# byvfx/go-raytracing

Hardware: AMD Instinct MI355X
Metric: Msamples/sec (pixels x SPP / s) (higher is better)
Workload: dtype f32; 1 GPU; cornell-lucy 1200x675 500spp depth 5; scene=cornell-lucy, width=1200, height=675, spp=500, max_depth=5, parallelism=tiles-rr1, buckets=836, blas=sah, nodes=fp32, triangles=280000, bvh_nodes=60240, bvh_nodes8=0, image_finite=True

## Files before the change

### go-raytracing_amd/__init__.py

```python
from __future__ import annotations

import ctypes as C
import os
from typing import Optional, Sequence

import numpy as np

PKG_DIR = os.path.dirname(os.path.abspath(__file__))
LIB_DIR = os.path.join(PKG_DIR, os.environ.get("RTGPU_LIB_DIR", "lib"))
REPO_DIR = os.path.dirname(PKG_DIR)
ASSET_DIR = os.path.join(REPO_DIR, "assets")

RT_OK = 0
RT_OPT_BLAS_BUILDER, RT_OPT_TLAS_BUILDER, RT_OPT_NODE_FORMAT = 1, 2, 3
RT_OPT_BATCH_SLOTS, RT_OPT_REFILL, RT_OPT_MAX_BLOCKS, RT_OPT_STREAMS = 4, 5, 6, 7
RT_OPT_VOLUMES = 8
RT_VOLUMES_LIFTED, RT_VOLUMES_IN_BVH = 0, 1
RT_OPT_BVH4_COLLAPSE = 9
RT_COLLAPSE_SAH, RT_COLLAPSE_GREEDY = 0, 1
RT_BLAS_REFERENCE, RT_BLAS_SAH, RT_BLAS_DEVICE = 0, 1, 2
RT_NODES_FP32, RT_NODES_QUANT8, RT_NODES_WIDE8 = 0, 1, 2
RT_OPT_DEALING, RT_OPT_DEAL_FIRST = 10, 11
RT_OPT_TAIL = 12
RT_OPT_OVERLAP = 13
RT_OPT_LIFT_PRIMS = 14
RT_PRIMS_LIFTED, RT_PRIMS_IN_BVH = 0, 1
RT_DEAL_STATIC, RT_DEAL_DYNAMIC = 0, 1
STATUS = {0: "RT_OK", -1: "RT_ERR_INVALID", -2: "RT_ERR_UNSUPPORTED", -3: "RT_ERR_HIP", -4: "RT_ERR_OOM",
          -5: "RT_ERR_NO_SCENE", -6: "RT_ERR_DEVICE"}

RT_SPHERE, RT_QUAD, RT_TRIANGLE, RT_PLANE, RT_LIST, RT_BVH_NODE, RT_BVH_LEAF = 1, 2, 3, 4, 5, 6, 7
RT_TRANSLATE, RT_ROTATE_X, RT_ROTATE_Y, RT_ROTATE_Z, RT_SCALE, RT_VOLUME = 8, 9, 10, 11, 12, 13
RT_CIRCLE = 14
RT_LAMBERTIAN, RT_METAL, RT_DIELECTRIC, RT_DIFFUSE_LIGHT, RT_ISOTROPIC = 1, 2, 3, 4, 5
RT_TEX_SOLID, RT_TEX_CHECKER, RT_TEX_NOISE, RT_TEX_IMAGE = 1, 2, 3, 4


class RtHittable(C.Structure):
    _fields_ = [("kind", C.c_int32), ("material", C.c_int32), ("a", C.c_int32), ("b", C.c_int32),
                ("bbox", C.c_double * 6), ("p", C.c_double * 16)]
# ... 149 lines not shown
        p.use_sky_gradient, p.phantom_hdri, p.camera_max_depth = camera.use_sky_gradient, camera.phantom_hdri, camera.max_depth
    for k, v in sky.items():
        if k == "background":
            p.background = (C.c_double * 3)(*[float(x) for x in v])
        elif k in ("use_sky_gradient", "phantom_hdri", "camera_max_depth"):
            setattr(p, k, int(v))
        else:
            raise TypeError(f"unknown rt_ray_color_params field {k!r}")
    return p


class RtWorkCounts(C.Structure):
    _fields_ = [(n, C.c_uint64) for n in ("samples", "rays", "shadow_rays", "node_visits", "sphere_tests",
                                          "quad_tests", "tri_tests", "plane_tests", "instance_visits",
                                          "volume_tests", "material_fetches", "env_lookups",
                                          "instance_box_tests", "stack_spills")]


class RtKernelTimes(C.Structure):
    _fields_ = [("extend_ms", C.c_double), ("shade_ms", C.c_double), ("shadow_ms", C.c_double),
                ("extend_launches", C.c_int32), ("shade_launches", C.c_int32), ("shadow_launches", C.c_int32),
                ("twins", C.c_int32)]


class RtSceneInfo(C.Structure):
    _fields_ = [(n, C.c_int32) for n in ("nodes", "leaves", "refs", "spheres", "quads", "triangles", "planes",
                                         "instances", "blases", "volumes", "materials", "textures", "lights",
                                         "stack_needed", "tlas_depth", "blas_depth")] + [("device_bytes", C.c_int64)] + \
        [("node_format", C.c_int32), ("nodes8", C.c_int32)]


# ... 557 lines not shown
    def set_collapse(self, collapse: str):
        self.set_option(RT_OPT_BVH4_COLLAPSE, {"sah": RT_COLLAPSE_SAH, "greedy": RT_COLLAPSE_GREEDY}[collapse])

    def set_schedule(self, batch_slots: int = 0, refill: int = 0, max_blocks: int = 0, streams: int = 0):
        self.set_option(RT_OPT_BATCH_SLOTS, batch_slots)
        self.set_option(RT_OPT_REFILL, refill)
        self.set_option(RT_OPT_MAX_BLOCKS, max_blocks)
        self.set_option(RT_OPT_STREAMS, streams)

    def set_tail(self, paths: int = 0):
        self.set_option(RT_OPT_TAIL, paths)

    def set_overlap(self, mode: int = 0):
        self.set_option(RT_OPT_OVERLAP, mode)

    def measure_read_bandwidth(self, nbytes: int = 4 << 30, reps: int = 10) -> float:
        gbs = C.c_double(0.0)
        self._check(self._lib.rt_measure_read_bandwidth(self._h, C.c_uint64(nbytes), reps, C.byref(gbs)))
        return float(gbs.value)

    def set_kernel_timing(self, enable: bool = True):
        self._check(self._lib.rt_set_kernel_timing(self._h, 1 if enable else 0))

    def last_kernel_times(self) -> dict:
        t = RtKernelTimes()
        self._check(self._lib.rt_last_kernel_times(self._h, C.byref(t)))
        return {n: getattr(t, n) for n, _ in RtKernelTimes._fields_}

    def tonemap(self, accum: np.ndarray, spp: int) -> np.ndarray:
        h, w = accum.shape[:2]
# ... 158 lines not shown
```

### go-raytracing_amd/csrc/api.cpp

```cpp
#include <hip/hip_runtime.h>

#include <algorithm>
#include <atomic>
#include <chrono>
#include <cstdio>
#include <cstdlib>
#include <cmath>
#include <cstring>
#include <string>
#include <thread>
#include <vector>

#include "../../include/rtgpu.h"
#include "dev_layout.h"
#include "build.h"
#include "flatten.h"
#include "probe.h"
#include "query.h"
#include "ray_source.h"
#include "wavefront.h"
#include "wave_layout.h"
#include "denoise.h"
#include "denoise_var.h"
#include "adaptive.h"
// ... 380 lines not shown
  hipStream_t sts[kMaxTwins] = {st};
  for (int t = 1; t < kMaxTwins; ++t) sts[t] = ctx->twin_st[t - 1];
  for (int t = 0; t < nt; ++t) {
    WaveArgs& a = as[t];
    bind_twin(a, static_cast<float4*>(ctx->wstate.p), static_cast<uint32_t*>(ctx->wq.p),
              static_cast<const uint32_t*>(ctx->wpix.p), static_cast<double*>(ctx->wacc.p),
              static_cast<uint32_t*>(ctx->wspill.p), lay.tw[t], lit);
    if (run.feat) feat_acc[t] = static_cast<double*>(ctx->wfacc.p) + lay.tw[t].pix_off * kFeatFloats;
    if (run.mom_out) mom_acc[t] = static_cast<double*>(ctx->wmacc.p) + lay.tw[t].pix_off * kMomFloats;
    a.seed = p->seed;
    a.max_depth = p->max_depth;
    a.counters = static_cast<unsigned long long*>(ctx->counters.p);
    a.err = static_cast<int*>(ctx->errflag.p);
    a.refill = knobs.refill;
    a.nee_probe = run.probing ? 1u : 0u;
    a.spill_lanes = spill.lanes;
    a.spill_cap = spill.cap;
    a.out_pixels = run.rays ? run.rays->num_rays : uint32_t(dc.width) * uint32_t(dc.height);
    ctx->twin_args[t] = a;
  }
  ctx->num_twins = nt;
  WavePlan plan{};
  plan.spp = spp;
  plan.samples_per_batch = bs.spb;
  plan.sample_offset = uint32_t(p->sample_offset);
  plan.max_depth = p->max_depth;
  if (run.feat) {
    plan.max_depth = 1;
    plan.feat_acc = feat_acc;
  }
// ... 371 lines not shown
    return RT_OK;
  }
  if (key == RT_OPT_REFILL) {
    if (value < 0 || value > 64) return set_err(ctx, RT_ERR_INVALID, "refill must be 0 (default) or 1..64");
    ctx->wopt.refill = value;
    return RT_OK;
  }
  if (key == RT_OPT_STREAMS) {
    if (value < 0 || value > kMaxTwins) return set_err(ctx, RT_ERR_INVALID, "streams must be 0 (default) or 1..4");
    ctx->wopt.streams = value;
    return RT_OK;
  }
  if (key == RT_OPT_OVERLAP) {
    if (value < 0 || value > 2) return set_err(ctx, RT_ERR_INVALID, "overlap must be 0 (default), 1 (off) or 2 (on)");
    ctx->wopt.overlap = value;
    return RT_OK;
  }
  if (key == RT_OPT_TAIL) {
    if (value < 0) return set_err(ctx, RT_ERR_INVALID, "bad tail option");
    ctx->wopt.tail = value;
    return RT_OK;
  }
  if (key == RT_OPT_MAX_BLOCKS) {
    if (value < 0) return set_err(ctx, RT_ERR_INVALID, "bad max blocks");
    ctx->wopt.blocks = value;
    return RT_OK;
  }
  if (key == RT_OPT_DEALING) {
    if (value != RT_DEAL_STATIC && value != RT_DEAL_DYNAMIC) return set_err(ctx, RT_ERR_INVALID, "bad dealing mode");
    ctx->opt_dealing = value;
// ... 783 lines not shown
void fill_counts(const unsigned long long* c, rt_work_counts* out) {
  out->samples = c[0];
  out->rays = c[1];
  out->shadow_rays = c[2];
  out->node_visits = c[3];
  out->sphere_tests = c[4];
  out->quad_tests = c[5];
  out->tri_tests = c[6];
  out->plane_tests = c[7];
  out->instance_visits = c[8];
  out->volume_tests = c[9];
  out->material_fetches = c[10];
  out->env_lookups = c[11];
  out->instance_box_tests = c[12];
  out->stack_spills = c[13];
}
}

int rt_count_work_by_kernel(rt_ctx* ctx, const rt_camera_desc* cam, const rt_render_params* params,
                            rt_work_counts* out) {
  if (!ctx || !cam || !out) return RT_ERR_INVALID;
  HIPCHK(hipSetDevice(ctx->device));
  unsigned long long c[CNT_WORDS] = {0};
  double ms = 0.0;
  int rc = render_impl(ctx, cam, params, nullptr, RenderRun{ctx->stream, &ms, c});
  if (rc) return rc;
  for (int k = 0; k < 3; ++k) fill_counts(c + k * CNT_BLOCK, out + k);
  return RT_OK;
}

// ... 473 lines not shown
```

### go-raytracing_amd/csrc/dev_layout.h

```cpp
#pragma once
#include <stdint.h>
#if !defined(__HIPCC__) && !defined(__host__)
#define __host__
#define __device__
#endif

namespace rtg {

enum : uint32_t {
  ITEM_NODE = 0u,
  ITEM_LEAF = 1u,
  ITEM_INSTANCE = 2u,
  ITEM_INST_END = 3u,
  ITEM_TRI1 = 4u,
  ITEM_WQUAD = 8u,
  ITEM_WSPHERE = 9u,
  ITEM_WINST = 10u,
  ITEM_LREF = 11u,
  ITEM_WTRI1 = 12u,
};
constexpr int ITEM_SHIFT = 28;
constexpr uint32_t ITEM_MASK = (1u << ITEM_SHIFT) - 1u;
constexpr int kInlineTriMax = 4;
__host__ __device__ inline uint32_t tri_leaf_item(uint32_t first, int n) {
// ... 300 lines not shown
  int32_t num_vol_refs;
  int32_t shade_kind;
  int32_t needs_uv;
  int32_t quant_nodes;
  int32_t dfs_order;
  int32_t wide_nodes;
  uint32_t root8;
  const DNode8* nodes8;
  const uint32_t* litems;
  const DWTri* wtris;
  uint32_t n_nodes, n_leaves, n_refs, n_spheres, n_quads, n_tris, n_instances, n_blas, n_volumes, n_circles;
  uint32_t n_nodes8, n_litems, n_wtris;
  int32_t num_prim_recs;
  const DPrimRec* prim_recs;
};

struct DCamera {
  float center[3];
  float pixel00[3];
  float du[3], dv[3];
  float disk_u[3], disk_v[3];
  float background[3];
  int32_t defocus;
  int32_t use_sky;
  int32_t phantom;
  int32_t cam_max_depth;
  int32_t width, height;
  int32_t slow, free_cam;
  float c_orig[3], c_dir[3];
  float la_orig[3], la_dir[3];
// ... 18 lines not shown
```

### go-raytracing_amd/csrc/device_common.h

```cpp
#pragma once
#include <hip/hip_runtime.h>
#include <stdint.h>
#include "dev_layout.h"

namespace rtg {

#ifdef RTG_GUARD
__device__ unsigned int rtg_guard_rec[4];
__device__ __forceinline__ void rtg_guard_note(int site, uint32_t i, uint32_t n) {
  if (atomicAdd(&rtg_guard_rec[0], 1u) == 0u) {
    rtg_guard_rec[1] = uint32_t(site);
    rtg_guard_rec[2] = i;
    rtg_guard_rec[3] = n;
  }
}
__device__ __forceinline__ uint32_t rtg_gix(uint32_t i, uint32_t n, int site) {
  if (i >= n) {
    rtg_guard_note(site, i, n);
    return n ? n - 1u : 0u;
  }
  return i;
}
#define GIX(i, n, site) rtg_gix(uint32_t(i), uint32_t(n), site)
#else
// ... 272 lines not shown
  const bool cc = closed_kind(kind), bc = closed_kind(bkind);
  if (cc != bc) return cc;
  const int rc = obj_rank(sc, refpos), rb = obj_rank(sc, brefpos);
  bool later;
  if (rc == rb) {
    if (primpos == bprimpos) return false;
    later = prim_rank(sc, kind, primpos) > prim_rank(sc, bkind, bprimpos);
  } else {
    later = rc > rb;
  }
  return cc ? later : !later;
}

struct Cnt {
  uint32_t rays, shadow, nodes, sph, quad, tri, plane, inst, vol, mat, env, ibox, spill;
};
__device__ __forceinline__ bool volume_flight(const DVolume& vol, V3 wd, bool h1, bool h2, float t1, float t2,
                                              float tmin, float tmax, int ntests, uint32_t key, uint32_t bounce,
                                              uint32_t dom, float& t_out) {
  if (!h1 || !h2) return false;
  if (t1 < tmin) t1 = tmin;
  if (t2 > tmax) t2 = tmax;
  if (t1 >= t2) return false;
  if (t1 < 0.0f) t1 = 0.0f;
  float rl = len(wd);
  float dist = (t2 - t1) * rl;
  float u = 0.0f;
  for (int p = 0; p < ntests; ++p) {
    float up = rnd(key, ctr(bounce, dom, uint32_t(vol.vol_id) * 4u + uint32_t(p)));
    u = up > u ? up : u;
// ... 363 lines not shown
  if (t < bt) return true;
  if (t == bt && bt < T.tmax) return tie_wins(sc, kind, refpos, primpos, S.hit_kind(), S.hit_refpos(), S.hit_primpos());
  return false;
}
__device__ __forceinline__ void take_hit(Trav& T, const TStack& S, float t, int kind, int idx, int refpos, int primpos) {
  T.bt = cull_widen(t);
  S.set_hit(kind, idx, refpos, primpos);
}
__device__ __forceinline__ Best trav_best(const Trav& T, const TStack& S) {
  Best b;
  b.t = best_t(T); b.inst = -1;
  b.kind = S.hit_kind(); b.idx = S.hit_idx(); b.refpos = S.hit_refpos(); b.primpos = S.hit_primpos();
  return b;
}

template <bool kAny, bool kCount, bool kWide = false>
__device__ __forceinline__ int trav_init(const DScene& sc, Trav& T, const TStack& S, V3 wo, V3 wd, float time,
                                         float tmin, float tmax, uint32_t key, uint32_t bounce, uint32_t voldom,
                                         Cnt& cnt) {
  S.set_time(time); T.tmin = tmin; T.tmax = tmax;
  T.key = key; T.bounce = bounce; T.voldom = voldom;
  T.bt = cull_widen(tmax);
  if (!kAny) S.set_hit(0, -1, 0, 0);
  for (int i = 0; i < sc.num_planes; ++i) {
    float t = 0.0f;
    if (kCount) cnt.plane++;
    if (plane_t(sc.planes[i], wo, wd, tmin, t)) {
      if (kAny) { if (t < tmax) return TRAV_ANYHIT; }
      else if (accept_hit(sc, t, PK_PLANE, -1 - i, 0, T, S)) take_hit(T, S, t, PK_PLANE, i, -1 - i, 0);
    }
  }
  T.cr = make_tray(wo, wd);
  S.save_world(wo, wd, T.cr.inv);
  S.set_cur_ref(-1); T.sp = 0;
  T.item = ITEM_NONE; T.lf = ITEM_NONE;
  float tn = 0.0f;
  if (sc.tlas.check_box &&
      !box_hit(sc.tlas.box[0], sc.tlas.box[1], sc.tlas.box[2], sc.tlas.box[3], sc.tlas.box[4], sc.tlas.box[5],
               T.cr, tmin, kAny ? tmax : T.bt, tn))
    return TRAV_DONE;
  T.item = kWide ? sc.root8 : sc.tlas.root_item;
  if ((T.item >> ITEM_SHIFT) != ITEM_NODE) {
    T.lf = T.item;
    T.item = item_is_leaf(T.lf) ? ITEM_NONE : ITEM_POP;
  }
  return TRAV_RUNNING;
}

template <bool kAny, bool kCount, bool kVol, bool kQuant = false, bool kWide = false, int kLdsN = 0>
__device__ __forceinline__ int trav_step(const DScene& sc, Trav& T, const TStack& S, Cnt& cnt, int* err) {
  const bool exact = kVol && !kAny && sc.dfs_order != 0;
  auto pop = [&]() -> uint32_t {
    for (;;) {
      if (T.sp == 0) return ITEM_NONE;
      --T.sp;
// ... 667 lines not shown
```

### go-raytracing_amd/csrc/wave_layout.h

```cpp
#pragma once
#include <algorithm>
#include <cstddef>
#include <cstdint>
#include <cstdlib>
#include <vector>

#include "wavefront.h"

namespace rtg {


struct WaveOptions {
  size_t slots = 0;
  int refill = 0;
  int blocks = 0;
  int tail = 0;
  int streams = 0;
  int overlap = 0;
};

struct WaveKnobs {
  int streams = 0;
  int overlap = 0;
  size_t slots = 0;
  int refill = 16;
  int max_blocks = 0;
  int debug_sync = 0;
  uint32_t tail_rays = 0;
  int tail_first = kTailFirstDefault;
};

struct WaveEnv {
  int streams, overlap, refill, max_blocks, tail_rays, tail_first, debug_sync;
  size_t slots;
};

inline WaveEnv read_wave_env() {
  auto num = [](const char* name, long unset) {
    const char* e = getenv(name);
    return e ? atol(e) : unset;
  };
  WaveEnv v{};
  v.streams = int(std::min<long>(kMaxTwins, std::max<long>(0, num("RTGPU_STREAMS", 0))));
  v.overlap = int(num("RTGPU_OVERLAP", 0));
  v.slots = size_t(std::max<long>(0, num("RTGPU_SLOTS", 0)));
  v.refill = int(std::min<long>(64, std::max<long>(1, num("RTGPU_REFILL", 16))));
  v.max_blocks = int(std::max<long>(0, num("RTGPU_MAX_BLOCKS", 0)));
  const long tail = num("RTGPU_TAIL_RAYS", -1);
  v.tail_rays = tail >= 0 ? int(tail) : kTailRaysDefault;
  v.tail_first = int(num("RTGPU_TAIL_FIRST", kTailFirstDefault));
  v.debug_sync = num("RTGPU_DEBUG_SYNC", 0) > 0 ? 1 : 0;
  return v;
}

inline const WaveEnv& wave_env() {
  static const WaveEnv env = read_wave_env();
  return env;
}

inline WaveKnobs resolve_knobs(const WaveOptions& opt, bool probing, const WaveEnv& env = wave_env()) {
  WaveKnobs k;
  k.streams = opt.streams ? opt.streams : env.streams;
  k.overlap = opt.overlap ? opt.overlap : env.overlap;
  k.slots = opt.slots ? opt.slots : env.slots;
  k.refill = opt.refill ? opt.refill : env.refill;
  k.max_blocks = opt.blocks ? opt.blocks : env.max_blocks;
  k.debug_sync = env.debug_sync;
  k.tail_rays = probing || opt.tail == 1 ? 0u : uint32_t(opt.tail > 1 ? opt.tail : env.tail_rays);
  k.tail_first = env.tail_first;
  return k;
}


constexpr int kDefaultTwins = 2;
constexpr uint64_t kThreeTwinSamples = uint64_t(1) << 26;
constexpr int kOverlapTwins = 2;

inline uint64_t tile_pixels(const std::vector<int4>& tiles) {
  uint64_t n = 0;
  for (const int4& tl : tiles) n += uint64_t(tl.z) * uint64_t(tl.w);
  return n;
}

inline bool use_overlap(const WaveKnobs& k, bool lit) { return lit && k.overlap == 2; }

inline int choose_twins(const WaveKnobs& k, bool shade_vol, bool overlap, uint64_t tile_px, int spp, size_t ntiles) {
  int automatic = shade_vol ? 1 : tile_px * uint64_t(std::max(1, spp)) > kThreeTwinSamples ? 3 : kDefaultTwins;
  if (overlap) automatic = std::min(automatic, kOverlapTwins);
  const int want = k.streams ? k.streams : automatic;
  return int(std::max<size_t>(1, std::min<size_t>(size_t(std::max(1, want)), ntiles)));
}

inline void deal_pixels(const std::vector<int4>& tiles, int width, int nt, std::vector<uint32_t>& out,
                        uint32_t twin_npix[kMaxTwins]) {
  out.clear();
  for (int t = 0; t < kMaxTwins; ++t) twin_npix[t] = 0;
  for (int t = 0; t < nt; ++t) {
    const size_t before = out.size();
    for (size_t k = size_t(t); k < tiles.size(); k += size_t(nt)) {
// ... 162 lines not shown
```

### go-raytracing_amd/csrc/wavefront.h

```cpp
#pragma once
#include <hip/hip_runtime.h>
#include <stdint.h>
#include "dev_layout.h"
#include "features.h"
#include "moments.h"

namespace rtg {

struct RaySource;

struct PathStream {
  float4* o;
  float4* d;
  float4* beta;
};

constexpr int kSlotF4 = 14;
constexpr int kSlotF4Dark = 8;

struct WaveArgs {
  PathStream s[2];
  float4* hit;
  float4* Lout;
  float4* sj_p;
// ... 8 lines not shown
  const uint32_t* pixels;
  uint32_t npix;
  double* acc;
  uint32_t seed;
  int32_t max_depth;
  unsigned long long* counters;
  int* err;
  int32_t refill;
  uint32_t nee_probe;
  uint32_t* spill;
  uint32_t* spill_sh;
  uint32_t spill_lanes;
  int32_t spill_cap;
  uint32_t slots;
  uint32_t out_pixels;
};

enum : int { CNT_STREAM0 = 0, CNT_STREAM1 = 32, CNT_SHADOW = 64, CNT_FETCH_EXT = 128, CNT_FETCH_SH = 384,
             CNT_SHADE_SEG = 896, CNT_WORDS_Q = 1152 };
__host__ __device__ constexpr int cnt_shadow(int parity) { return CNT_SHADOW + 32 * parity; }
__host__ __device__ constexpr int cnt_fetch_sh(int parity) { return CNT_FETCH_SH + 256 * parity; }

constexpr int kLdsStack = 8;
constexpr int kStackMax = 128;
constexpr int kSpillLanesPerCU = 2048;

constexpr int kTailRaysDefault = 1 << 23;
constexpr int kTailFirstDefault = 7;

struct WavePlan {
  uint32_t tail_rays;
  int32_t tail_first;
  uint32_t spp;
  uint32_t samples_per_batch;
// ... 7 lines not shown
  const hipStream_t* aux;
  const hipEvent_t* ev_shade;
  const hipEvent_t* ev_nee;
  uint32_t* probe_host;
  int* bounces_run;
  hipEvent_t* events;
  uint8_t* ev_class;
  int max_events;
  int* num_events;
  double* const* feat_acc;
  double* const* mom_acc;
  float* mom_out;
  const RaySource* ray_src;
};

enum : uint8_t { KC_EXTEND = 0, KC_SHADE = 1, KC_SHADOW = 2, KC_OTHER = 3 };
constexpr int KC_TWIN_SHIFT = 4;
constexpr int kMaxTwins = 4;
constexpr int CNT_BLOCK = 24;

#ifdef RTG_GUARD
hipError_t guard_report(unsigned int out[4]);
#endif
hipError_t launch_wavefront(const DScene& sc, const DCamera& cam, const WaveArgs* as, const hipStream_t* sts,
                            const WavePlan& plan, bool count, float* out, int accumulate);

}
```

### go-raytracing_amd/csrc/wavefront.hip

```cpp
#include <hip/hip_runtime.h>
#include <stdint.h>
#include <stdio.h>
#include <type_traits>

#include "dev_layout.h"
#include "device_common.h"
#include "wave_variant.h"
#include "wavefront.h"
#include "ray_source.h"

namespace rtg {

constexpr int kTravWaves = 7, kVolWaves = 4;
#define TRAV_WAVES(kVol, kCount) ((kCount) ? 4 : (kVol) ? kVolWaves : kTravWaves)
constexpr int kLdsNodesExt = 4, kLdsNodesSh = 20, kLdsNodesTail = 64;
constexpr int lds_nodes_for(int k, bool kQuant, bool kWide) { return (kQuant || kWide) ? 0 : k; }
constexpr int lds_node_rows(int k) { return k > 0 ? k * 8 : 1; }

__device__ __forceinline__ float asf(uint32_t u) { return __uint_as_float(u); }
__device__ __forceinline__ uint32_t asu(float f) { return __float_as_uint(f); }

#ifdef RTG_HOST_EMU
__device__ __forceinline__ float4 ldnt(const float4* p) { return *p; }
__device__ __forceinline__ void stnt(float4* p, float4 v) { *p = v; }
// ... 10 lines not shown
  __builtin_nontemporal_store(w, reinterpret_cast<rtg_v4f*>(p));
}
__device__ __forceinline__ uint32_t ldnt(const uint32_t* p) { return __builtin_nontemporal_load(p); }
__device__ __forceinline__ void stnt(uint32_t* p, uint32_t v) { __builtin_nontemporal_store(v, p); }
#endif

__device__ __forceinline__ uint32_t pack_state(int depth, uint32_t bounce, bool allow) {
  return uint32_t(depth & 0xFFFF) | ((bounce & 0x7FFFu) << 16) | (allow ? 0x80000000u : 0u);
}

__device__ __forceinline__ uint32_t lanes_below(unsigned long long m) {
  return uint32_t(__popcll(m & ((1ull << __lane_id()) - 1ull)));
}

__device__ __forceinline__ void add_counters(unsigned long long* c, const Cnt& n, uint32_t samples) {
  const uint32_t f[13] = {n.rays, n.shadow, n.nodes, n.sph, n.quad, n.tri, n.plane, n.inst, n.vol, n.mat, n.env, n.ibox, n.spill};
  atomicAdd(c, (unsigned long long)samples);
  for (int k = 0; k < 13; ++k) atomicAdd(c + 1 + k, (unsigned long long)f[k]);
}

__device__ __forceinline__ uint32_t slot_pixel(const WaveArgs& a, uint32_t i) {
  return a.pixels[GIX(i % a.npix, a.npix, 51)];
}
__device__ __forceinline__ void camera_ray(const DCamera& cam, const WaveArgs& a, uint32_t i, uint32_t pix,
                                           uint32_t sample_base, V3& ro, V3& rd, uint32_t& key) {
  const int px = int(pix % uint32_t(cam.width)), py = int(pix / uint32_t(cam.width));
  key = path_key(a.seed, pix, sample_base + i / a.npix);
  float time;
  get_ray(cam, px, py, key, ro, rd, time);
}

constexpr uint32_t kGssDiv = 4;
constexpr uint32_t kSegs = 8;
// ... 136 lines not shown
__device__ __forceinline__ void block_reserve2(bool c0, bool c1, uint32_t* q0, uint32_t* q1, uint32_t (*sw)[4],
                                               uint32_t* sb, uint32_t& p0, uint32_t& p1) {
  const unsigned long long m0 = __ballot(c0), m1 = __ballot(c1);
  const int w = int(threadIdx.x >> 6);
  if (__lane_id() == 0) { sw[0][w] = uint32_t(__popcll(m0)); sw[1][w] = uint32_t(__popcll(m1)); }
  __syncthreads();
  for (uint32_t q = threadIdx.x; q < 2u; q += blockDim.x) {
    const int nw = int((blockDim.x + 63u) >> 6);
    uint32_t tot = 0;
    for (int k = 0; k < nw; ++k) { const uint32_t c = sw[q][k]; sw[q][k] = tot; tot += c; }
    sb[q] = tot ? atomicAdd(q ? q1 : q0, tot) : 0u;
  }
  __syncthreads();
  p0 = sb[0] + sw[0][w] + lanes_below(m0);
  p1 = sb[1] + sw[1][w] + lanes_below(m1);
}

__device__ __forceinline__ uint32_t shade_claim(uint32_t* ctr, uint32_t nchunks, uint32_t& seg, uint32_t& tried) {
  for (;;) {
    const uint32_t lo = uint32_t((uint64_t(nchunks) * seg) / kSegs), hi = uint32_t((uint64_t(nchunks) * (seg + 1u)) / kSegs);
    const uint32_t c = atomicAdd(ctr + seg * kSegStride, 1u);
    if (lo + c < hi) return lo + c;
    if (++tried >= kSegs) return 0xFFFFFFFFu;
    seg = (seg + 1u) & (kSegs - 1u);
  }
}

template <bool kCount, bool kEnvIS, int kShadeL, bool kFirst>
__device__ __forceinline__ void shade_path(const DScene& sc, const DCamera& cam, const WaveArgs& a, const DVolRec* vrecs,
                                           const float4 h, const V3 ro, const V3 rd, const V3 beta, const uint32_t key,
// ... 207 lines not shown

constexpr int kShadeFullWaves = 4, kShadeLeanWaves = 7, kShadeMatWaves = 7, kShadeVolWaves = 6;
#define SHADE_WAVES(kShadeL)                                                    \
  (((kShadeL) & SHADE_KIND_MASK) == SHADE_FULL ? kShadeFullWaves                 \
   : ((kShadeL) & SHADE_KIND_MASK) == SHADE_MAT ? kShadeMatWaves                 \
   : ((kShadeL) & SHADE_KIND_MASK) == SHADE_VOL ? kShadeVolWaves : kShadeLeanWaves)
template <bool kCount, bool kEnvIS, int kShadeL, bool kFirst>
static __global__ __launch_bounds__(256, SHADE_WAVES(kShadeL)) void k_shade(DScene scg, DCamera cam, WaveArgs a, PathStream cs,
                                               const uint32_t* count, PathStream ns, uint32_t* ncount,
                                               uint32_t* jcount, uint32_t sample_base, uint32_t launch_bounce) {
#ifdef RTG_HOST_EMU
  static char s_dyn[kLdsMaterials * sizeof(DMaterial) + kLdsTextures * sizeof(DTexture) + kLdsLights * sizeof(DLight)];
#else
  extern __shared__ char s_dyn[];
#endif
  __shared__ uint32_t s_w[2][2][4];
  __shared__ uint32_t s_b[2][2];
  constexpr int kShade = kShadeL & SHADE_KIND_MASK;
  DScene sc = scg;
  const DVolRec* const vrecs = sc.vol_recs;
  constexpr bool kLdsTables = kShade != SHADE_FULL;
  if (kLdsTables || shade_tables_fit(sc)) shade_tables_to_lds(sc, s_dyn);
  const uint32_t n = *count;
  const uint32_t gs = gridDim.x * blockDim.x;
  if (blockIdx.x == 0 && threadIdx.x == 0)
    for (uint32_t k = 0; k < kSegs; ++k) a.counts[CNT_FETCH_EXT + k * kSegStride] = 0u;
  Cnt cnt = {};
  const uint32_t n_up = (n + 255u) & ~255u;
  uint32_t par = 0;
  (void)gs;
  __shared__ uint32_t s_chunk[2];
  uint32_t seg = xcc_id(), tried = 0;
  const uint32_t nchunks = n_up / blockDim.x;
  if (threadIdx.x == 0) s_chunk[0] = shade_claim(a.counts + CNT_SHADE_SEG, nchunks, seg, tried);
  for (;; par ^= 1u) {
    __syncthreads();
    const uint32_t chunk = s_chunk[par];
    if (chunk == 0xFFFFFFFFu) break;
    const uint32_t i = chunk * blockDim.x + threadIdx.x;
    const bool live = i < n;
    bool cont = false, want_shadow = false;
    uint32_t slot = 0, key = 0, flags = 0, bounce = 0, nstate = 0;
    float tmax_a = 0.0f;
    V3 P = mk(0.0f, 0.0f, 0.0f), sd = P, beta = P, nbeta = P, ca = P, ch = P, da = P, dh = P;
    bool lout_set = false;
    if (live) {
      if (kCount) cnt.rays++;
      const uint32_t ii = GIX(i, a.slots, 41);
      const float4 h = ldnt(&a.hit[ii]);
      if (threadIdx.x == 0) s_chunk[par ^ 1u] = shade_claim(a.counts + CNT_SHADE_SEG, nchunks, seg, tried);
      V3 ro, rd;
      int dleft;
      bool allow;
      if (kFirst) {
        slot = ii;
        camera_ray(cam, a, ii, slot_pixel(a, ii), sample_base, ro, rd, key);
        dleft = a.max_depth;
        bounce = 0;
        allow = true;
        beta = mk(1.0f, 1.0f, 1.0f);
      } else {
        const float4 o4 = ldnt(&cs.o[ii]), d4 = ldnt(&cs.d[ii]), b4 = ldnt(&cs.beta[ii]);
        key = asu(d4.w);
        slot = asu(o4.w);
// ... 1 lines not shown
        dleft = int(st & 0xFFFFu);
        bounce = launch_bounce;
#ifdef RTG_GUARD
        if (((st >> 16) & 0x7FFFu) != launch_bounce) rtg_guard_note(52, (st >> 16) & 0x7FFFu, launch_bounce);
#endif
        allow = (st >> 31) != 0u;
        ro = mk(o4.x, o4.y, o4.z);
        rd = mk(d4.x, d4.y, d4.z);
        beta = mk(b4.x, b4.y, b4.z);
      }
      shade_path<kCount, kEnvIS, kShadeL, kFirst>(sc, cam, a, vrecs, h, ro, rd, beta, key, slot, dleft, bounce, allow, cont,
                                                 want_shadow, flags, nstate, tmax_a, P, sd, nbeta, ca, ch, da, dh,
                                                 lout_set, cnt);
    }
    if (!live && threadIdx.x == 0) s_chunk[par ^ 1u] = shade_claim(a.counts + CNT_SHADE_SEG, nchunks, seg, tried);
    if (kFirst && live && !lout_set) stnt(&a.Lout[GIX(slot, a.slots, 44)], make_float4(0.0f, 0.0f, 0.0f, 0.0f));
    uint32_t jc = 0, js = 0;
    block_reserve2(cont, want_shadow, ncount, jcount, s_w[par], s_b[par], jc, js);
    if (cont) {
      jc = GIX(jc, a.slots, 43);
      stnt(&ns.o[jc], make_float4(P.x, P.y, P.z, asf(slot)));
      stnt(&ns.d[jc], make_float4(sd.x, sd.y, sd.z, asf(key)));
      stnt(&ns.beta[jc], make_float4(nbeta.x, nbeta.y, nbeta.z, asf(nstate)));
    }
    if (want_shadow) {
      if (kCount) cnt.shadow++;
      js = GIX(js, a.slots, 45);
      stnt(&a.sj_p[js], make_float4(P.x, P.y, P.z, asf(key)));
      stnt(&a.sj_a[js], make_float4(da.x, da.y, da.z, tmax_a));
      if (kEnvIS) stnt(&a.sj_h[js], make_float4(dh.x, dh.y, dh.z, 0.0f));
      stnt(&a.sj_info[js], flags | (bounce << 8));
      if (kEnvIS) {
        stnt(&a.ne_a[js], make_float4(ca.x, ca.y, ca.z, asf(slot)));
// ... 207 lines not shown
}

static __global__ __launch_bounds__(256) void k_finalize(WaveArgs a, float* out, int accumulate) {
  const uint32_t gs = gridDim.x * blockDim.x;
  for (uint32_t pi = blockIdx.x * blockDim.x + threadIdx.x; pi < a.npix; pi += gs) {
    float* o = out + size_t(GIX(a.pixels[pi], a.out_pixels, 58)) * 3;
    double sx = a.acc[size_t(pi) * 3], sy = a.acc[size_t(pi) * 3 + 1], sz = a.acc[size_t(pi) * 3 + 2];
    if (accumulate) { sx += double(o[0]); sy += double(o[1]); sz += double(o[2]); }
    o[0] = float(sx); o[1] = float(sy); o[2] = float(sz);
  }
}

static __global__ void k_set_counts(uint32_t* c, uint32_t n) {
  if (threadIdx.x == 0) {
    c[CNT_STREAM0] = n; c[CNT_STREAM1] = 0u; c[cnt_shadow(0)] = 0u; c[cnt_shadow(1)] = 0u;
    for (uint32_t k = 0; k < kSegs; ++k) {
      c[CNT_FETCH_EXT + k * kSegStride] = 0u;
      c[cnt_fetch_sh(0) + k * kSegStride] = 0u;
      c[cnt_fetch_sh(1) + k * kSegStride] = 0u;
      c[CNT_SHADE_SEG + k * kSegStride] = 0u;
    }
  }
}

static __global__ void k_count_samples(WaveArgs a, uint32_t n) {
  if (blockIdx.x == 0 && threadIdx.x == 0) atomicAdd(a.counters, (unsigned long long)n);
}

#ifndef RTG_HOST_EMU
static int grid_for(const void* fn, int block, size_t lds, uint32_t items, int cus) {
// ... 139 lines not shown
          if (ovl) {
            if ((e = hipEventRecord(plan.ev_shade[t], st)) != hipSuccess) return e;
            if ((e = hipStreamWaitEvent(sx, plan.ev_shade[t], 0)) != hipSuccess) return e;
          }
          if ((e = mark_begin(plan, uint8_t(KC_SHADOW | (t << KC_TWIN_SHIFT)), sx)) != hipSuccess) return e;
          hipLaunchKernelGGL(k.shadow, dim3(gsd[t]), dim3(256), 0, sx, sc, a,
                             cnt_sh, fetch_sh, a.counts + cnt_fetch_sh(nx));
          if ((e = mark_end(plan, sx)) != hipSuccess) return e;
          RTG_LAUNCHED("k_shadow", b, sx);
          hipLaunchKernelGGL(k.nee_apply, dim3(gap[t]), dim3(256), 0, sx, a, cnt_sh);
          RTG_LAUNCHED("k_nee_apply", b, sx);
          if (ovl && (e = hipEventRecord(plan.ev_nee[t], sx)) != hipSuccess) return e;
        }
      }
      if (plan.max_depth > 8 && ((b >= 7 && (b % 4) == 3) || (plan.tail_rays > 0 && b == plan.tail_first))) {
        for (int t = 0; t < nt; ++t)
          if ((e = hipMemcpyAsync(plan.probe_host + t, as[t].counts + (nx ? CNT_STREAM1 : CNT_STREAM0), sizeof(uint32_t),
                                  hipMemcpyDeviceToHost, sts[t])) != hipSuccess)
            return e;
        uint32_t left = 0;
        uint32_t lefts[kMaxTwins] = {};
        for (int t = 0; t < nt; ++t) {
          if ((e = hipStreamSynchronize(sts[t])) != hipSuccess) return e;
          left += plan.probe_host[t];
          lefts[t] = plan.probe_host[t];
          const int need = int((plan.probe_host[t] + 255u) / 256u);
          const int g = need < kSegs ? int(kSegs) : need;
          if (g < gext[t]) gext[t] = g;
          if (g < gsd[t]) gsd[t] = g;
          if (g < gsh[t]) gsh[t] = g;
        }
        if (left == 0) break;
        if (k.tail != nullptr && !nee && plan.tail_rays > 0 && left <= plan.tail_rays && b + 1 < plan.max_depth) {
          const size_t lds = shade_lds_bytes(sc);
          const int cap_tail = int(as[0].spill_lanes / 256u);
          for (int t = 0; t < nt; ++t) {
            if (lefts[t] == 0) continue;
            const WaveArgs& a = as[t];
// ... 121 lines not shown
```

### go/rtgpu/rtgpu.go

```go
package rtgpu

import "C"

import (
	"errors"
	"fmt"
	"runtime"
	"unsafe"
)

const ABIVersion = 8

const (
	KindSphere    int32 = 1
	KindQuad      int32 = 2
	KindTriangle  int32 = 3
	KindPlane     int32 = 4
	KindList      int32 = 5
	KindBVHNode   int32 = 6
	KindBVHLeaf   int32 = 7
	KindTranslate int32 = 8
	KindRotateX   int32 = 9
	KindRotateY   int32 = 10
	KindRotateZ   int32 = 11
// ... 40 lines not shown
	VolumesInBVH    int32 = 1
	OptBVH4Collapse int32 = 9
	CollapseSAH     int32 = 0
	CollapseGreedy  int32 = 1
	BuildReference  int32 = 0
	BuildSAH        int32 = 1
	BuildDevice     int32 = 2
	NodesFP32       int32 = 0
	NodesQuant8     int32 = 1
	NodesWide8      int32 = 2
	OptDealing      int32 = 10
	OptDealFirst    int32 = 11
	OptTail         int32 = 12
	OptOverlap      int32 = 13
	OptLiftPrims    int32 = 14
	PrimsLifted     int32 = 0
	PrimsInBVH      int32 = 1
	DealStatic      int32 = 0
	DealDynamic     int32 = 1
)

type Node struct {
	Kind     int32       `c:"kind"`
	Material int32       `c:"material"`
	A        int32       `c:"a"`
	B        int32       `c:"b"`
	BBox     [6]float64  `c:"bbox"`
	P        [16]float64 `c:"p"`
}

// ... 669 lines not shown
```

### include/rtgpu.h

```cpp
#ifndef RTGPU_H
#define RTGPU_H

#include <stddef.h>
#include <stdint.h>

#ifdef __cplusplus
extern "C" {
#endif

#define RT_ABI_VERSION 8

enum rt_status {
  RT_OK = 0,
  RT_ERR_INVALID = -1,
  RT_ERR_UNSUPPORTED = -2,
  RT_ERR_HIP = -3,
  RT_ERR_OOM = -4,
  RT_ERR_NO_SCENE = -5,
  RT_ERR_DEVICE = -6
};

enum rt_hittable_kind {
  RT_SPHERE = 1,
  RT_QUAD = 2,
// ... 132 lines not shown
typedef struct rt_stats {
  double kernel_ms;
  uint64_t samples;
} rt_stats;

typedef struct rt_work_counts {
  uint64_t samples;
  uint64_t rays;
  uint64_t shadow_rays;
  uint64_t node_visits;
  uint64_t sphere_tests, quad_tests, tri_tests, plane_tests;
  uint64_t instance_visits, volume_tests;
  uint64_t material_fetches, env_lookups;
  uint64_t instance_box_tests;
  uint64_t stack_spills;
} rt_work_counts;

typedef struct rt_kernel_times {
  double extend_ms, shade_ms, shadow_ms;
  int32_t extend_launches, shade_launches, shadow_launches, twins;
} rt_kernel_times;

typedef struct rt_scene_info {
  int32_t nodes, leaves, refs, spheres, quads, triangles, planes;
  int32_t instances, blases, volumes, materials, textures, lights;
  int32_t stack_needed, tlas_depth, blas_depth;
  int64_t device_bytes;
  int32_t node_format;
  int32_t nodes8;
} rt_scene_info;
// ... 3 lines not shown
int rt_abi_version(void);

int rt_ctx_create(int device, rt_ctx** out);
void rt_ctx_destroy(rt_ctx* ctx);
const char* rt_last_error(const rt_ctx* ctx);

int rt_device_count(int32_t* num_devices);

int rt_ctx_create_multi(const int32_t* devices, int32_t num_devices, rt_ctx** out);
int rt_ctx_num_devices(const rt_ctx* ctx);
int rt_last_dealing(const rt_ctx* ctx, int32_t* tiles, int32_t* runs, int32_t max_devices);

enum { RT_OPT_BLAS_BUILDER = 1, RT_OPT_TLAS_BUILDER = 2, RT_OPT_NODE_FORMAT = 3,
       RT_OPT_BATCH_SLOTS = 4, RT_OPT_REFILL = 5, RT_OPT_MAX_BLOCKS = 6, RT_OPT_STREAMS = 7,
       RT_OPT_VOLUMES = 8, RT_OPT_BVH4_COLLAPSE = 9, RT_OPT_DEALING = 10, RT_OPT_DEAL_FIRST = 11,
       RT_OPT_TAIL = 12, RT_OPT_OVERLAP = 13, RT_OPT_LIFT_PRIMS = 14 };
enum { RT_PRIMS_LIFTED = 0, RT_PRIMS_IN_BVH = 1 };
enum { RT_DEAL_STATIC = 0, RT_DEAL_DYNAMIC = 1 };
enum { RT_BLAS_REFERENCE = 0, RT_BLAS_SAH = 1, RT_BLAS_DEVICE = 2 };
enum { RT_NODES_FP32 = 0, RT_NODES_QUANT8 = 1, RT_NODES_WIDE8 = 2 };
enum { RT_VOLUMES_LIFTED = 0, RT_VOLUMES_IN_BVH = 1 };
enum { RT_COLLAPSE_SAH = 0, RT_COLLAPSE_GREEDY = 1 };
int rt_ctx_set_option(rt_ctx* ctx, int32_t key, int32_t value);

int rt_scene_upload(rt_ctx* ctx, const rt_scene_desc* scene);

int rt_scene_get_info(const rt_ctx* ctx, rt_scene_info* out);

int rt_scene_lifted_prims(const rt_ctx* ctx, int32_t* count);

int rt_last_build_ms(const rt_ctx* ctx, double* ms);
// ... 141 lines not shown
```

Measured before the change: 2316 Msamples/s.

## Resolve world-box misses in shade kernel, skipping shadow and extend launches

In the shade kernel, shadow rays whose segment misses the world bounding box are resolved on the spot: their light contribution is added to Lout and no shadow ray is queued. Continuation rays that miss the world box go to a separate back-of-buffer queue, and the next shade pass treats them as misses without running the extend traversal. This cuts queue traffic and traversal work for rays that obviously escape the scene. In exchange it adds a three-way block reservation, extra counters, and extra host probe copies. It only applies when the scene has a TLAS world box, no planes and lifted primitives, and the cornell-lucy scene is closed, so few rays may leave the box.

```diff
diff --git a/go-raytracing_amd/__init__.py b/go-raytracing_amd/__init__.py
--- a/go-raytracing_amd/__init__.py
+++ b/go-raytracing_amd/__init__.py
@@ -24,6 +24,7 @@
 RT_OPT_TAIL = 12
 RT_OPT_OVERLAP = 13
 RT_OPT_LIFT_PRIMS = 14
+RT_OPT_EARLY_MISS = 15
 RT_PRIMS_LIFTED, RT_PRIMS_IN_BVH = 0, 1
 RT_DEAL_STATIC, RT_DEAL_DYNAMIC = 0, 1
 STATUS = {0: "RT_OK", -1: "RT_ERR_INVALID", -2: "RT_ERR_UNSUPPORTED", -3: "RT_ERR_HIP", -4: "RT_ERR_OOM",
@@ -203,7 +204,8 @@
     _fields_ = [(n, C.c_uint64) for n in ("samples", "rays", "shadow_rays", "node_visits", "sphere_tests",
                                           "quad_tests", "tri_tests", "plane_tests", "instance_visits",
                                           "volume_tests", "material_fetches", "env_lookups",
-                                          "instance_box_tests", "stack_spills")]
+                                          "instance_box_tests", "stack_spills", "early_shadow_rays",
+                                          "early_rays")]
 
 
 class RtKernelTimes(C.Structure):
@@ -791,6 +793,9 @@
     def set_overlap(self, mode: int = 0):
         self.set_option(RT_OPT_OVERLAP, mode)
 
+    def set_early_miss(self, mode: int = 0):
+        self.set_option(RT_OPT_EARLY_MISS, mode)
+
     def measure_read_bandwidth(self, nbytes: int = 4 << 30, reps: int = 10) -> float:
         gbs = C.c_double(0.0)
         self._check(self._lib.rt_measure_read_bandwidth(self._h, C.c_uint64(nbytes), reps, C.byref(gbs)))
diff --git a/go-raytracing_amd/csrc/api.cpp b/go-raytracing_amd/csrc/api.cpp
--- a/go-raytracing_amd/csrc/api.cpp
+++ b/go-raytracing_amd/csrc/api.cpp
@@ -418,6 +418,7 @@
     a.err = static_cast<int*>(ctx->errflag.p);
     a.refill = knobs.refill;
     a.nee_probe = run.probing ? 1u : 0u;
+    a.early_miss = early_miss_bits(knobs, early_miss_eligible(ctx->dscene), run.probing, lit, p->max_depth);
     a.spill_lanes = spill.lanes;
     a.spill_cap = spill.cap;
     a.out_pixels = run.rays ? run.rays->num_rays : uint32_t(dc.width) * uint32_t(dc.height);
@@ -819,6 +820,11 @@
   if (key == RT_OPT_OVERLAP) {
     if (value < 0 || value > 2) return set_err(ctx, RT_ERR_INVALID, "overlap must be 0 (default), 1 (off) or 2 (on)");
     ctx->wopt.overlap = value;
+    return RT_OK;
+  }
+  if (key == RT_OPT_EARLY_MISS) {
+    if (value < 0 || value > 2) return set_err(ctx, RT_ERR_INVALID, "early miss must be 0 (default), 1 (off) or 2 (on)");
+    ctx->wopt.early_miss = value;
     return RT_OK;
   }
   if (key == RT_OPT_TAIL) {
@@ -1632,6 +1638,8 @@
   out->env_lookups = c[11];
   out->instance_box_tests = c[12];
   out->stack_spills = c[13];
+  out->early_shadow_rays = c[14];
+  out->early_rays = c[15];
 }
 }
 
diff --git a/go-raytracing_amd/csrc/dev_layout.h b/go-raytracing_amd/csrc/dev_layout.h
--- a/go-raytracing_amd/csrc/dev_layout.h
+++ b/go-raytracing_amd/csrc/dev_layout.h
@@ -338,6 +338,8 @@
   int32_t num_prim_recs;
   const DPrimRec* prim_recs;
 };
+__host__ __device__ inline bool world_box_decides(const DScene& sc) { return sc.tlas.check_box != 0 && sc.num_planes == 0; }
+__host__ __device__ inline bool early_miss_eligible(const DScene& sc) { return world_box_decides(sc) && sc.num_prim_recs > 0; }
 
 struct DCamera {
   float center[3];
diff --git a/go-raytracing_amd/csrc/device_common.h b/go-raytracing_amd/csrc/device_common.h
--- a/go-raytracing_amd/csrc/device_common.h
+++ b/go-raytracing_amd/csrc/device_common.h
@@ -310,6 +310,8 @@
 
 struct Cnt {
   uint32_t rays, shadow, nodes, sph, quad, tri, plane, inst, vol, mat, env, ibox, spill;
+  uint32_t early_nee;
+  uint32_t early_next;
 };
 __device__ __forceinline__ bool volume_flight(const DVolume& vol, V3 wd, bool h1, bool h2, float t1, float t2,
                                               float tmin, float tmax, int ntests, uint32_t key, uint32_t bounce,
@@ -703,6 +705,15 @@
   return b;
 }
 
+__device__ __forceinline__ bool world_box_missed(const DScene& sc, const TRay& r, float tmin, float hi) {
+  float tn = 0.0f;
+  return !box_hit(sc.tlas.box[0], sc.tlas.box[1], sc.tlas.box[2], sc.tlas.box[3], sc.tlas.box[4], sc.tlas.box[5], r, tmin,
+                  hi, tn);
+}
+__device__ __forceinline__ bool world_box_missed(const DScene& sc, V3 o, V3 d, float tmin, float hi) {
+  return world_box_missed(sc, make_tray(o, d), tmin, hi);
+}
+
 template <bool kAny, bool kCount, bool kWide = false>
 __device__ __forceinline__ int trav_init(const DScene& sc, Trav& T, const TStack& S, V3 wo, V3 wd, float time,
                                          float tmin, float tmax, uint32_t key, uint32_t bounce, uint32_t voldom,
@@ -723,11 +734,7 @@
   S.save_world(wo, wd, T.cr.inv);
   S.set_cur_ref(-1); T.sp = 0;
   T.item = ITEM_NONE; T.lf = ITEM_NONE;
-  float tn = 0.0f;
-  if (sc.tlas.check_box &&
-      !box_hit(sc.tlas.box[0], sc.tlas.box[1], sc.tlas.box[2], sc.tlas.box[3], sc.tlas.box[4], sc.tlas.box[5],
-               T.cr, tmin, kAny ? tmax : T.bt, tn))
-    return TRAV_DONE;
+  if (sc.tlas.check_box && world_box_missed(sc, T.cr, tmin, kAny ? tmax : T.bt)) return TRAV_DONE;
   T.item = kWide ? sc.root8 : sc.tlas.root_item;
   if ((T.item >> ITEM_SHIFT) != ITEM_NODE) {
     T.lf = T.item;
diff --git a/go-raytracing_amd/csrc/wave_layout.h b/go-raytracing_amd/csrc/wave_layout.h
--- a/go-raytracing_amd/csrc/wave_layout.h
+++ b/go-raytracing_amd/csrc/wave_layout.h
@@ -17,6 +17,7 @@
   int tail = 0;
   int streams = 0;
   int overlap = 0;
+  int early_miss = 0;
 };
 
 struct WaveKnobs {
@@ -28,11 +29,13 @@
   int debug_sync = 0;
   uint32_t tail_rays = 0;
   int tail_first = kTailFirstDefault;
+  int early_miss = 0;
 };
 
 struct WaveEnv {
   int streams, overlap, refill, max_blocks, tail_rays, tail_first, debug_sync;
   size_t slots;
+  int early_miss;
 };
 
 inline WaveEnv read_wave_env() {
@@ -50,6 +53,7 @@
   v.tail_rays = tail >= 0 ? int(tail) : kTailRaysDefault;
   v.tail_first = int(num("RTGPU_TAIL_FIRST", kTailFirstDefault));
   v.debug_sync = num("RTGPU_DEBUG_SYNC", 0) > 0 ? 1 : 0;
+  v.early_miss = int(num("RTGPU_EARLY_MISS", 0));
   return v;
 }
 
@@ -68,6 +72,7 @@
   k.debug_sync = env.debug_sync;
   k.tail_rays = probing || opt.tail == 1 ? 0u : uint32_t(opt.tail > 1 ? opt.tail : env.tail_rays);
   k.tail_first = env.tail_first;
+  k.early_miss = opt.early_miss ? opt.early_miss : env.early_miss;
   return k;
 }
 
@@ -83,6 +88,12 @@
 }
 
 inline bool use_overlap(const WaveKnobs& k, bool lit) { return lit && k.overlap == 2; }
+
+inline uint32_t early_miss_bits(const WaveKnobs& k, bool eligible, bool probing, bool lit, int max_depth) {
+  if (k.early_miss == 1 || !eligible || probing) return 0u;
+  const bool may_tail = !lit && k.tail_rays > 0 && max_depth > 8;
+  return EARLY_NEE | (may_tail ? 0u : EARLY_NEXT);
+}
 
 inline int choose_twins(const WaveKnobs& k, bool shade_vol, bool overlap, uint64_t tile_px, int spp, size_t ntiles) {
   int automatic = shade_vol ? 1 : tile_px * uint64_t(std::max(1, spp)) > kThreeTwinSamples ? 3 : kDefaultTwins;
diff --git a/go-raytracing_amd/csrc/wavefront.h b/go-raytracing_amd/csrc/wavefront.h
--- a/go-raytracing_amd/csrc/wavefront.h
+++ b/go-raytracing_amd/csrc/wavefront.h
@@ -46,10 +46,12 @@
   int32_t spill_cap;
   uint32_t slots;
   uint32_t out_pixels;
+  uint32_t early_miss;
 };
 
 enum : int { CNT_STREAM0 = 0, CNT_STREAM1 = 32, CNT_SHADOW = 64, CNT_FETCH_EXT = 128, CNT_FETCH_SH = 384,
-             CNT_SHADE_SEG = 896, CNT_WORDS_Q = 1152 };
+             CNT_SHADE_SEG = 896, CNT_BACK = 1152, CNT_WORDS_Q = 1248 };
+__host__ __device__ constexpr int cnt_back(uint32_t bounce) { return CNT_BACK + 32 * int(bounce % 3u); }
 __host__ __device__ constexpr int cnt_shadow(int parity) { return CNT_SHADOW + 32 * parity; }
 __host__ __device__ constexpr int cnt_fetch_sh(int parity) { return CNT_FETCH_SH + 256 * parity; }
 
@@ -87,6 +89,7 @@
   const RaySource* ray_src;
 };
 
+enum : uint32_t { EARLY_NEE = 1u, EARLY_NEXT = 2u };
 enum : uint8_t { KC_EXTEND = 0, KC_SHADE = 1, KC_SHADOW = 2, KC_OTHER = 3 };
 constexpr int KC_TWIN_SHIFT = 4;
 constexpr int kMaxTwins = 4;
diff --git a/go-raytracing_amd/csrc/wavefront.hip b/go-raytracing_amd/csrc/wavefront.hip
--- a/go-raytracing_amd/csrc/wavefront.hip
+++ b/go-raytracing_amd/csrc/wavefront.hip
@@ -48,9 +48,10 @@
 }
 
 __device__ __forceinline__ void add_counters(unsigned long long* c, const Cnt& n, uint32_t samples) {
-  const uint32_t f[13] = {n.rays, n.shadow, n.nodes, n.sph, n.quad, n.tri, n.plane, n.inst, n.vol, n.mat, n.env, n.ibox, n.spill};
+  const uint32_t f[15] = {n.rays, n.shadow, n.nodes, n.sph, n.quad, n.tri, n.plane, n.inst, n.vol, n.mat, n.env, n.ibox, n.spill,
+                          n.early_nee, n.early_next};
   atomicAdd(c, (unsigned long long)samples);
-  for (int k = 0; k < 13; ++k) atomicAdd(c + 1 + k, (unsigned long long)f[k]);
+  for (int k = 0; k < 15; ++k) atomicAdd(c + 1 + k, (unsigned long long)f[k]);
 }
 
 __device__ __forceinline__ uint32_t slot_pixel(const WaveArgs& a, uint32_t i) {
@@ -217,6 +218,26 @@
   __syncthreads();
   p0 = sb[0] + sw[0][w] + lanes_below(m0);
   p1 = sb[1] + sw[1][w] + lanes_below(m1);
+}
+
+__device__ __forceinline__ void block_reserve3(bool c0, bool cb, bool c1, uint32_t* q0, uint32_t* qb, uint32_t* q1,
+                                               uint32_t slots, uint32_t (*sw)[4], uint32_t* sb, uint32_t& p0, uint32_t& pb,
+                                               uint32_t& p1) {
+  const unsigned long long m0 = __ballot(c0), mb = __ballot(cb), m1 = __ballot(c1);
+  const int w = int(threadIdx.x >> 6);
+  if (__lane_id() == 0) { sw[0][w] = uint32_t(__popcll(m0)); sw[1][w] = uint32_t(__popcll(mb)); sw[2][w] = uint32_t(__popcll(m1)); }
+  __syncthreads();
+  for (uint32_t q = threadIdx.x; q < 3u; q += blockDim.x) {
+    const int nw = int((blockDim.x + 63u) >> 6);
+    uint32_t tot = 0;
+    for (int k = 0; k < nw; ++k) { const uint32_t c = sw[q][k]; sw[q][k] = tot; tot += c; }
+    const uint32_t base = tot ? atomicAdd(q == 0u ? q0 : q == 1u ? qb : q1, tot) : 0u;
+    sb[q] = q == 1u ? slots - (base + tot) : base;
+  }
+  __syncthreads();
+  p0 = sb[0] + sw[0][w] + lanes_below(m0);
+  pb = sb[1] + sw[1][w] + lanes_below(mb);
+  p1 = sb[2] + sw[2][w] + lanes_below(m1);
 }
 
 __device__ __forceinline__ uint32_t shade_claim(uint32_t* ctr, uint32_t nchunks, uint32_t& seg, uint32_t& tried) {
@@ -454,31 +475,39 @@
 #else
   extern __shared__ char s_dyn[];
 #endif
-  __shared__ uint32_t s_w[2][2][4];
-  __shared__ uint32_t s_b[2][2];
   constexpr int kShade = kShadeL & SHADE_KIND_MASK;
+  constexpr bool kEarly = (kShadeL & SHADE_LIFT) != 0;
+  __shared__ uint32_t s_w[2][kEarly ? 3 : 2][4];
+  __shared__ uint32_t s_b[2][kEarly ? 3 : 2];
   DScene sc = scg;
   const DVolRec* const vrecs = sc.vol_recs;
   constexpr bool kLdsTables = kShade != SHADE_FULL;
   if (kLdsTables || shade_tables_fit(sc)) shade_tables_to_lds(sc, s_dyn);
   const uint32_t n = *count;
   const uint32_t gs = gridDim.x * blockDim.x;
-  if (blockIdx.x == 0 && threadIdx.x == 0)
+  const bool back = kEarly && (a.early_miss & EARLY_NEXT) != 0u;
+  const uint32_t nb = (back && !kFirst) ? a.counts[cnt_back(launch_bounce)] : 0u;
+  uint32_t* const bcount = a.counts + cnt_back(launch_bounce + 1u);
+  if (blockIdx.x == 0 && threadIdx.x == 0) {
     for (uint32_t k = 0; k < kSegs; ++k) a.counts[CNT_FETCH_EXT + k * kSegStride] = 0u;
+    if (back) a.counts[cnt_back(launch_bounce + 2u)] = 0u;
+  }
   Cnt cnt = {};
   const uint32_t n_up = (n + 255u) & ~255u;
   uint32_t par = 0;
   (void)gs;
   __shared__ uint32_t s_chunk[2];
   uint32_t seg = xcc_id(), tried = 0;
-  const uint32_t nchunks = n_up / blockDim.x;
+  const uint32_t fchunks = n_up / blockDim.x;
+  const uint32_t nchunks = fchunks + ((nb + 255u) & ~255u) / blockDim.x;
   if (threadIdx.x == 0) s_chunk[0] = shade_claim(a.counts + CNT_SHADE_SEG, nchunks, seg, tried);
   for (;; par ^= 1u) {
     __syncthreads();
     const uint32_t chunk = s_chunk[par];
     if (chunk == 0xFFFFFFFFu) break;
-    const uint32_t i = chunk * blockDim.x + threadIdx.x;
-    const bool live = i < n;
+    const bool bchunk = kEarly && chunk >= fchunks;
+    const uint32_t i = (bchunk ? chunk - fchunks : chunk) * blockDim.x + threadIdx.x;
+    const bool live = i < (bchunk ? nb : n);
     bool cont = false, want_shadow = false;
     uint32_t slot = 0, key = 0, flags = 0, bounce = 0, nstate = 0;
     float tmax_a = 0.0f;
@@ -486,8 +515,8 @@
     bool lout_set = false;
     if (live) {
       if (kCount) cnt.rays++;
-      const uint32_t ii = GIX(i, a.slots, 41);
-      const float4 h = ldnt(&a.hit[ii]);
+      const uint32_t ii = GIX(bchunk ? a.slots - nb + i : i, a.slots, 41);
+      const float4 h = bchunk ? make_float4(__builtin_inff(), 0.0f, asf(0xFFFFFFFFu), 0.0f) : ldnt(&a.hit[ii]);
       if (threadIdx.x == 0) s_chunk[par ^ 1u] = shade_claim(a.counts + CNT_SHADE_SEG, nchunks, seg, tried);
       V3 ro, rd;
       int dleft;
@@ -519,9 +548,39 @@
                                                  lout_set, cnt);
     }
     if (!live && threadIdx.x == 0) s_chunk[par ^ 1u] = shade_claim(a.counts + CNT_SHADE_SEG, nchunks, seg, tried);
+    bool early = false;
+    float4 l4 = make_float4(0.0f, 0.0f, 0.0f, 0.0f);
+    if (kEarly && (a.early_miss & EARLY_NEE) && want_shadow) {
+      early = !(flags & 1u) || world_box_missed(sc, P, da, 0.001f, tmax_a);
+      if (kEnvIS && (flags & 2u)) early = early && world_box_missed(sc, P, dh, 0.001f, __builtin_inff());
+      if (early) {
+        want_shadow = false;
+        lout_set = true;
+        if (!kFirst) l4 = ldnt(&a.Lout[GIX(slot, a.slots, 44)]);
+        if (kCount) cnt.early_nee += (flags & 1u) + ((flags >> 1) & 1u);
+      }
+    }
     if (kFirst && live && !lout_set) stnt(&a.Lout[GIX(slot, a.slots, 44)], make_float4(0.0f, 0.0f, 0.0f, 0.0f));
-    uint32_t jc = 0, js = 0;
-    block_reserve2(cont, want_shadow, ncount, jcount, s_w[par], s_b[par], jc, js);
+    const bool cback = back && cont && world_box_missed(sc, P, sd, 0.001f, cull_widen(__builtin_inff()));
+    if (kCount && cback) cnt.early_next++;
+    uint32_t jc = 0, jb = 0, js = 0;
+    if constexpr (kEarly) {
+      block_reserve3(cont && !cback, cback, want_shadow, ncount, bcount, jcount, a.slots, s_w[par], s_b[par], jc, jb, js);
+      if (cback) jc = jb;
+    } else {
+      block_reserve2(cont, want_shadow, ncount, jcount, s_w[par], s_b[par], jc, js);
+    }
+    if (early) {
+      V3 direct = mul(beta, ca);
+      if (kEnvIS) {
+        direct = mk(0.0f, 0.0f, 0.0f);
+        if (flags & 2u) direct = add(direct, ch);
+        if (flags & 1u) direct = add(direct, ca);
+        direct = mul(beta, direct);
+      }
+      const V3 L = add(mk(l4.x, l4.y, l4.z), direct);
+      stnt(&a.Lout[GIX(slot, a.slots, 44)], make_float4(L.x, L.y, L.z, 0.0f));
+    }
     if (cont) {
       jc = GIX(jc, a.slots, 43);
       stnt(&ns.o[jc], make_float4(P.x, P.y, P.z, asf(slot)));
@@ -759,6 +818,7 @@
 static __global__ void k_set_counts(uint32_t* c, uint32_t n) {
   if (threadIdx.x == 0) {
     c[CNT_STREAM0] = n; c[CNT_STREAM1] = 0u; c[cnt_shadow(0)] = 0u; c[cnt_shadow(1)] = 0u;
+    for (uint32_t k = 0; k < 3u; ++k) c[cnt_back(k)] = 0u;
     for (uint32_t k = 0; k < kSegs; ++k) {
       c[CNT_FETCH_EXT + k * kSegStride] = 0u;
       c[cnt_fetch_sh(0) + k * kSegStride] = 0u;
@@ -928,14 +988,21 @@
         }
       }
       if (plan.max_depth > 8 && ((b >= 7 && (b % 4) == 3) || (plan.tail_rays > 0 && b == plan.tail_first))) {
-        for (int t = 0; t < nt; ++t)
+        for (int t = 0; t < nt; ++t) {
           if ((e = hipMemcpyAsync(plan.probe_host + t, as[t].counts + (nx ? CNT_STREAM1 : CNT_STREAM0), sizeof(uint32_t),
                                   hipMemcpyDeviceToHost, sts[t])) != hipSuccess)
             return e;
+          plan.probe_host[kMaxTwins + t] = 0u;
+          if ((as[t].early_miss & EARLY_NEXT) &&
+              (e = hipMemcpyAsync(plan.probe_host + kMaxTwins + t, as[t].counts + cnt_back(uint32_t(b) + 1u), sizeof(uint32_t),
+                                  hipMemcpyDeviceToHost, sts[t])) != hipSuccess)
+            return e;
+        }
         uint32_t left = 0;
         uint32_t lefts[kMaxTwins] = {};
         for (int t = 0; t < nt; ++t) {
           if ((e = hipStreamSynchronize(sts[t])) != hipSuccess) return e;
+          plan.probe_host[t] += plan.probe_host[kMaxTwins + t];
           left += plan.probe_host[t];
           lefts[t] = plan.probe_host[t];
           const int need = int((plan.probe_host[t] + 255u) / 256u);
diff --git a/go/rtgpu/rtgpu.go b/go/rtgpu/rtgpu.go
--- a/go/rtgpu/rtgpu.go
+++ b/go/rtgpu/rtgpu.go
@@ -78,6 +78,7 @@
 	OptTail         int32 = 12
 	OptOverlap      int32 = 13
 	OptLiftPrims    int32 = 14
+	OptEarlyMiss    int32 = 15
 	PrimsLifted     int32 = 0
 	PrimsInBVH      int32 = 1
 	DealStatic      int32 = 0
diff --git a/include/rtgpu.h b/include/rtgpu.h
--- a/include/rtgpu.h
+++ b/include/rtgpu.h
@@ -170,6 +170,8 @@
   uint64_t material_fetches, env_lookups;
   uint64_t instance_box_tests;
   uint64_t stack_spills;
+  uint64_t early_shadow_rays;
+  uint64_t early_rays;
 } rt_work_counts;
 
 typedef struct rt_kernel_times {
@@ -203,7 +205,8 @@
 enum { RT_OPT_BLAS_BUILDER = 1, RT_OPT_TLAS_BUILDER = 2, RT_OPT_NODE_FORMAT = 3,
        RT_OPT_BATCH_SLOTS = 4, RT_OPT_REFILL = 5, RT_OPT_MAX_BLOCKS = 6, RT_OPT_STREAMS = 7,
        RT_OPT_VOLUMES = 8, RT_OPT_BVH4_COLLAPSE = 9, RT_OPT_DEALING = 10, RT_OPT_DEAL_FIRST = 11,
-       RT_OPT_TAIL = 12, RT_OPT_OVERLAP = 13, RT_OPT_LIFT_PRIMS = 14 };
+       RT_OPT_TAIL = 12, RT_OPT_OVERLAP = 13, RT_OPT_LIFT_PRIMS = 14,
+       RT_OPT_EARLY_MISS = 15 };
 enum { RT_PRIMS_LIFTED = 0, RT_PRIMS_IN_BVH = 1 };
 enum { RT_DEAL_STATIC = 0, RT_DEAL_DYNAMIC = 1 };
 enum { RT_BLAS_REFERENCE = 0, RT_BLAS_SAH = 1, RT_BLAS_DEVICE = 2 };
```

Measured after the change: 2601 Msamples/s, median of 6. 12.3% higher.
